# D-Hank/NeRF-tiny

Hardware: AMD Instinct MI355X
Metric: rays/sec (64 coarse + 128 fine samples), lego 400x400 (higher is better)
Workload: dtype f32

## Files before the change

### nerf-tiny_amd/csrc/field_fwd_reg.hip

```cpp
#include "field_common.h"

namespace nerf {

constexpr int RM = 32;

template <int NFT>
struct WStage {
  float4 w[NFT];
};

template <int KB, int NFT>
__device__ __forceinline__ void stage_load(const float4* __restrict__ seg_lane, int kb, WStage<NFT>& s) {
#pragma unroll
  for (int f = 0; f < NFT; ++f) s.w[f] = seg_lane[(size_t)(f * KB + kb) * 64];
}

__device__ __forceinline__ float relu1(float x) { return __int_as_float(max(__float_as_int(x), 0)); }

__device__ __forceinline__ float f4c(const float4& v, int c) { return c == 0 ? v.x : (c == 1 ? v.y : (c == 2 ? v.z : v.w)); }

struct SaveIn {
  float* rows;
  uint16_t* mask;
};

template <int KB, int NFT, int NKB, int NNFT, bool ZERO_INIT, bool RELU_IN, int SAVE = 0>
__device__ __forceinline__ void reg_layer(const int seg, const int next_seg , int lane,
                                          const f32x16* prev, f32x16* acc, WStage<8>& st0, const float* bv,
                                          const SaveIn sv, const RegBuf& rb) {
  constexpr int KT = KB / 4;
  WStage<8> st1;
  const f32x16 zero = {0.f, 0.f, 0.f, 0.f, 0.f, 0.f, 0.f, 0.f, 0.f, 0.f, 0.f, 0.f, 0.f, 0.f, 0.f, 0.f};
  if (bv != nullptr) {
    const float one_h0 = (lane < 32) ? 1.0f : 0.0f;
#pragma unroll
    for (int f = 0; f < NFT; ++f) acc[f] = __builtin_amdgcn_mfma_f32_32x32x2f32(bv[f], one_h0, zero, 0, 0, 0);
  }
  f32x16 tin[2];
  auto activate = [&](int t) {
#pragma unroll
    for (int r = 0; r < 16; ++r) tin[t & 1][r] = RELU_IN ? (SAVE == 1 ? fmaxf(prev[t][r], 0.f) : relu1(prev[t][r])) : prev[t][r];
#pragma unroll
    for (int r = 0; r < 16; ++r) asm volatile("" : "+v"(tin[t & 1][r]));
    if (SAVE == 1 || (SAVE == 2 && !RELU_IN)) {
#pragma unroll
      for (int g = 0; g < 4; ++g)
        store_row4(sv.rows + 32 * t + 8 * g, make_float4(tin[t & 1][4 * g], tin[t & 1][4 * g + 1], tin[t & 1][4 * g + 2], tin[t & 1][4 * g + 3]));
    }
    if (SAVE != 0 && RELU_IN) {
      unsigned bits = 0;
#pragma unroll
      for (int r = 0; r < 16; ++r) bits |= (prev[t][r] > 0.f) ? (1u << r) : 0u;
      sv.mask[((t & 1) * 2) * 256 + (t >> 1) * 64] = (uint16_t)bits;
    }
  };
  activate(0);
#pragma unroll
  for (int kb = 0; kb < KB; ++kb) {
    WStage<8>& ld = (kb & 1) ? st0 : st1;
    const WStage<8>& cur = (kb & 1) ? st1 : st0;
    if (kb + 1 < KB) {
#pragma unroll
      for (int f = 0; f < NFT; ++f) ld.w[f] = reg_ldw(rb, seg + (f * KB + kb + 1) * 64);
    } else if (next_seg >= 0) {
#pragma unroll
      for (int f = 0; f < NNFT; ++f) ld.w[f] = reg_ldw(rb, next_seg + (f * NKB) * 64);
    }
    __builtin_amdgcn_sched_barrier(0);
    if ((kb & 3) == 2 && (kb >> 2) + 1 < KT) activate((kb >> 2) + 1);
#pragma unroll
    for (int s = 0; s < 4; ++s) {
      const float b = tin[(kb >> 2) & 1][4 * (kb & 3) + s];
#pragma unroll
      for (int f = 0; f < NFT; ++f) {
        if (ZERO_INIT && bv == nullptr && kb == 0 && s == 0)
          acc[f] = __builtin_amdgcn_mfma_f32_32x32x2f32(f4c(cur.w[f], s), b, zero, 0, 0, 0);
        else
          acc[f] = __builtin_amdgcn_mfma_f32_32x32x2f32(f4c(cur.w[f], s), b, acc[f], 0, 0, 0);
      }
    }
  }
  if (KB & 1) st0 = st1;
}

template <int NFT>
__device__ __forceinline__ void bias_load(const float* __restrict__ bias, int lane, float (&bv)[8]) {
#pragma unroll
  for (int f = 0; f < NFT; ++f) bv[f] = bias[f * 32 + (lane & 31)];
}

#ifdef NERF_STAMPS
#define RSTAMP(slot)                                            \
  do {                                                          \
    __builtin_amdgcn_sched_barrier(0);                          \
    const unsigned long long t_ = __builtin_readcyclecounter(); \
    __builtin_amdgcn_sched_barrier(0);                          \
    tsum[slot] += t_ - tlast;                                   \
    tlast = t_;                                                 \
  } while (0)
#else
#define RSTAMP(slot) do { } while (0)
#endif

enum { SRC_RAYS = 0, SRC_POINTS = 1, SRC_LATTICE = 2 };

template <bool SAVE, bool DEBUG, int SRC = SRC_RAYS, bool RGB = true, bool GSAVE = false>
__global__ __launch_bounds__(64, 1) void k_field_fwd_reg(const FieldArgs a, const QuerySrc q) {
#ifdef NERF_STAMPS
  unsigned long long tsum[12] = {0, 0, 0, 0, 0, 0, 0, 0, 0, 0, 0, 0};
  unsigned long long tlast = __builtin_readcyclecounter();
#endif
  const int lane = threadIdx.x, j = lane & 31, h = lane >> 5;
  const int m0 = blockIdx.x * RM;
  const int m = m0 + j;
  const bool valid = m < a.M;
  const int mc = valid ? m : a.M - 1;
  const int ray = (SRC == SRC_RAYS) ? mc / a.N : mc;
  const float* rf = (SRC == SRC_RAYS) ? a.rayf + (size_t)ray * RAYF : nullptr;
  const float4* wp = a.wp;
  const RegBuf rb = reg_buf(a.wp, threadIdx.x);

  WStage<8> st0;
  stage_load<8, 8>(wp + seg_off4(SEG_L0) + lane, 0, st0);

  float p[3];
  if constexpr (SRC == SRC_RAYS) {
    sample_point(rf, a.t[mc], p);
  } else if constexpr (SRC == SRC_POINTS) {
#pragma unroll
    for (int c = 0; c < 3; ++c) p[c] = q.points[(size_t)mc * 3 + c];
  } else {
    const int iz = mc % q.nz, ixy = mc / q.nz;
    const int iy = ixy % q.ny, ix = ixy / q.ny;
    p[0] = q.lo[0] + (float)ix * q.step[0];
    p[1] = q.lo[1] + (float)iy * q.step[1];
    p[2] = q.lo[2] + (float)iz * q.step[2];
  }
  if (DEBUG && a.pts_dbg && valid && h == 0) {
    a.pts_dbg[(size_t)m * 3 + 0] = p[0];
    a.pts_dbg[(size_t)m * 3 + 1] = p[1];
    a.pts_dbg[(size_t)m * 3 + 2] = p[2];
  }
  f32x16 gp[2];
#pragma unroll
  for (int g8 = 0; g8 < 8; ++g8) {
#pragma unroll
    for (int e = 0; e < 2; ++e) {
      const int pi = 4 * g8 + 2 * h + e;
      float sv = 0.f, cv = 0.f;
      if (pi < 30) {
        const int c = pi / 10, l = pi - 10 * c;
        const float x = (c == 0) ? p[0] : ((c == 1) ? p[1] : p[2]);
        const float ph = x * __uint_as_float(kFreqPointBits[l]);
        sincos_phase(ph, sv, cv);
      }
      gp[g8 >> 2][4 * (g8 & 3) + 2 * e] = sv;
      gp[g8 >> 2][4 * (g8 & 3) + 2 * e + 1] = cv;
    }
  }
  if (DEBUG && a.gp_dbg && valid) {
#pragma unroll
    for (int g8 = 0; g8 < 8; ++g8)
#pragma unroll
      for (int s = 0; s < 4; ++s) {
        const int k = 8 * g8 + 4 * h + s;
        if (k < POINT_DIM) a.gp_dbg[(size_t)m * POINT_DIM + k] = gp[g8 >> 2][4 * (g8 & 3) + s];
      }
  }

  const size_t MS = (size_t)a.MSrows * WIDTH;
  const long long rrow = valid ? (long long)(a.row0 + m) : a.Mtot + j;
  float* const srow = SAVE ? a.save + (size_t)rrow * WIDTH + 4 * h : nullptr;
  uint16_t* const mrow = (SAVE || GSAVE) ? a.masks + ((size_t)(a.tile0 + (m0 >> 6)) * 4 + ((m0 >> 5) & 1)) * 256 + h * 32 + j : nullptr;
  const size_t MKS = (size_t)a.tiles_tot * 4 * 256;
  auto sv_rows = [&](int tensor) { return SaveIn{SAVE ? srow + (size_t)tensor * MS : nullptr, nullptr}; };
  auto sv_relu = [&](int layer) { return SaveIn{SAVE ? srow + (size_t)layer * MS : nullptr, SAVE ? mrow + (size_t)layer * MKS : nullptr}; };
  float* const gprow = GSAVE ? a.save + (size_t)rrow * QGRAD_GP + 4 * h : nullptr;
  float* const crow = GSAVE ? a.save + (size_t)a.MSrows * QGRAD_GP + (size_t)rrow * QGRAD_C + 4 * h : nullptr;
  constexpr int SV = SAVE ? 1 : (GSAVE ? 2 : 0);
  auto sv_in = [&](int layer) { return GSAVE ? SaveIn{nullptr, mrow + (size_t)layer * MKS} : sv_relu(layer); };

  RSTAMP(0);
  f32x16 A[8], B[8];
  constexpr int L256 = 8 * 32 * 64;
  constexpr int sL1 = seg_off4(SEG_L1);
  constexpr int sL5 = seg_off4(SEG_L5);
  float bv[8];

  bias_load<8>(a.w.p[B_L0], lane, bv);
  reg_layer<8, 8, 32, 8, true, false, SV>(seg_off4(SEG_L0), sL1, lane, gp, A, st0, bv, GSAVE ? SaveIn{gprow, nullptr} : sv_rows(S_GP), rb);
  RSTAMP(1);
  bias_load<8>(a.w.p[3], lane, bv);
  reg_layer<32, 8, 32, 8, true, true, SV>(sL1, sL1 + L256, lane, A, B, st0, bv, sv_in(0), rb);
  bias_load<8>(a.w.p[5], lane, bv);
  reg_layer<32, 8, 32, 8, true, true, SV>(sL1 + L256, sL1 + 2 * L256, lane, B, A, st0, bv, sv_in(1), rb);
  bias_load<8>(a.w.p[7], lane, bv);
  reg_layer<32, 8, 32, 8, true, true, SV>(sL1 + 2 * L256, seg_off4(SEG_L4A), lane, A, B, st0, bv, sv_in(2), rb);
  RSTAMP(2);
  bias_load<8>(a.w.p[9], lane, bv);
  reg_layer<32, 8, 8, 8, true, true, SV>(seg_off4(SEG_L4A), seg_off4(SEG_L4B), lane, B, A, st0, bv, sv_in(3), rb);
  reg_layer<8, 8, 32, 8, false, false>(seg_off4(SEG_L4B), sL5, lane, gp, A, st0, nullptr, SaveIn{nullptr, nullptr}, rb);
  RSTAMP(3);
  bias_load<8>(a.w.p[11], lane, bv);
  reg_layer<32, 8, 32, 8, true, true, SV>(sL5, sL5 + L256, lane, A, B, st0, bv, sv_in(4), rb);
  bias_load<8>(a.w.p[13], lane, bv);
  reg_layer<32, 8, 32, 8, true, true, SV>(sL5 + L256, sL5 + 2 * L256, lane, B, A, st0, bv, sv_in(5), rb);
  bias_load<8>(a.w.p[15], lane, bv);
  reg_layer<32, 8, 32, 4, true, true, SV>(sL5 + 2 * L256, RGB ? seg_off4(SEG_FOLD) : -1, lane, A, B, st0, bv, sv_in(6), rb);
  RSTAMP(4);
  {
    const float* ws = a.w.p[W_SIGMA] + 4 * h;
    float s = 0.f;
    float4 wq[2][4];
#pragma unroll
    for (int g = 0; g < 4; ++g) wq[0][g] = *reinterpret_cast<const float4*>(ws + 8 * g);
#pragma unroll
    for (int t = 0; t < 8; ++t) {
      if (t + 1 < 8) {
#pragma unroll
        for (int g = 0; g < 4; ++g) wq[(t + 1) & 1][g] = *reinterpret_cast<const float4*>(ws + 32 * (t + 1) + 8 * g);
      }
      if (SAVE) __builtin_amdgcn_sched_barrier(0);
      if (GSAVE) {
        unsigned bits = 0;
#pragma unroll
        for (int r = 0; r < 16; ++r) bits |= (B[t][r] > 0.f) ? (1u << r) : 0u;
        mrow[7 * MKS + ((t & 1) * 2) * 256 + (t >> 1) * 64] = (uint16_t)bits;
      }
#pragma unroll
      for (int g = 0; g < 4; ++g) {
        const float4 q = wq[t & 1][g];
        s = __builtin_fmaf(relu1(B[t][4 * g + 0]), q.x, s);
        s = __builtin_fmaf(relu1(B[t][4 * g + 1]), q.y, s);
        s = __builtin_fmaf(relu1(B[t][4 * g + 2]), q.z, s);
        s = __builtin_fmaf(relu1(B[t][4 * g + 3]), q.w, s);
      }
      if (SAVE) __builtin_amdgcn_sched_barrier(0);
    }
    s += __shfl_xor(s, 32);
    if (valid && h == 0) {
      const float pre = s + a.w.p[B_SIGMA][0];
      a.sigma[m] = fabsf(pre);
      if (SAVE || GSAVE) a.spre[a.row0 + m] = pre;
    }
  }
  RSTAMP(5);
  if constexpr (!RGB) return;
  {
    const float* dv = a.dvec + (size_t)ray * HALF + 4 * h;
#pragma unroll
    for (int f = 0; f < 4; ++f)
#pragma unroll
      for (int g = 0; g < 4; ++g) {
        const float4 q = *reinterpret_cast<const float4*>(dv + 32 * f + 8 * g);
        A[f][4 * g + 0] = q.x;
        A[f][4 * g + 1] = q.y;
        A[f][4 * g + 2] = q.z;
        A[f][4 * g + 3] = q.w;
      }
  }
  reg_layer<32, 4, 32, 4, false, true, SAVE>(seg_off4(SEG_FOLD), -1, lane, B, A, st0, nullptr, GSAVE ? SaveIn{nullptr, nullptr} : sv_relu(7), rb);
  RSTAMP(6);
  {
    const float* wc = a.w.p[W_COLOR] + 4 * h;
    float z0 = 0.f, z1 = 0.f, z2 = 0.f;
#pragma unroll
    for (int t = 0; t < 4; ++t)
#pragma unroll
      for (int g = 0; g < 4; ++g) {
        const float4 q0 = *reinterpret_cast<const float4*>(wc + 32 * t + 8 * g);
        const float4 q1 = *reinterpret_cast<const float4*>(wc + HALF + 32 * t + 8 * g);
        const float4 q2 = *reinterpret_cast<const float4*>(wc + 2 * HALF + 32 * t + 8 * g);
        const float c0 = relu1(A[t][4 * g + 0]), c1 = relu1(A[t][4 * g + 1]);
        const float c2 = relu1(A[t][4 * g + 2]), c3 = relu1(A[t][4 * g + 3]);
        if (SAVE) store_row4(srow + S_C * MS + 32 * t + 8 * g, make_float4(c0, c1, c2, c3));
        if (GSAVE) store_row4(crow + 32 * t + 8 * g, make_float4(c0, c1, c2, c3));
        z0 = __builtin_fmaf(c3, q0.w, __builtin_fmaf(c2, q0.z, __builtin_fmaf(c1, q0.y, __builtin_fmaf(c0, q0.x, z0))));
        z1 = __builtin_fmaf(c3, q1.w, __builtin_fmaf(c2, q1.z, __builtin_fmaf(c1, q1.y, __builtin_fmaf(c0, q1.x, z1))));
        z2 = __builtin_fmaf(c3, q2.w, __builtin_fmaf(c2, q2.z, __builtin_fmaf(c1, q2.y, __builtin_fmaf(c0, q2.x, z2))));
      }
    z0 += __shfl_xor(z0, 32);
    z1 += __shfl_xor(z1, 32);
    z2 += __shfl_xor(z2, 32);
    if (valid && h == 0) {
      const float* bc = a.w.p[B_COLOR];
      a.rgb[(size_t)m * 3 + 0] = 1.0f / (1.0f + expf(-(z0 + bc[0])));
      a.rgb[(size_t)m * 3 + 1] = 1.0f / (1.0f + expf(-(z1 + bc[1])));
      a.rgb[(size_t)m * 3 + 2] = 1.0f / (1.0f + expf(-(z2 + bc[2])));
    }
  }
#ifdef NERF_STAMPS
  RSTAMP(7);
  if (a.stamps && lane == 0) {
    for (int i = 0; i < 8; ++i) atomicAdd(a.stamps + i, tsum[i]);
    atomicAdd(a.stamps + 31, 1ull);
  }
#endif
}

hipError_t launch_field_fwd_reg(const FieldArgs& a, bool save, hipStream_t st) {
  const int tiles = (a.M + RM - 1) / RM;
  if (save)
    hipLaunchKernelGGL((k_field_fwd_reg<true, false>), dim3(tiles), dim3(64), 0, st, a, QuerySrc{});
  else if (a.pts_dbg || a.gp_dbg)
    hipLaunchKernelGGL((k_field_fwd_reg<false, true>), dim3(tiles), dim3(64), 0, st, a, QuerySrc{});
  else
    hipLaunchKernelGGL((k_field_fwd_reg<false, false>), dim3(tiles), dim3(64), 0, st, a, QuerySrc{});
  return hipGetLastError();
}

hipError_t launch_query_grad_fwd(const FieldArgs& a, const QuerySrc& q, bool rgb, hipStream_t st) {
  if (a.M <= 0) return hipSuccess;
  const unsigned tiles = (unsigned)(((long long)a.M + RM - 1) / RM);
  if (rgb)
    hipLaunchKernelGGL((k_field_fwd_reg<false, false, SRC_POINTS, true, true>), dim3(tiles), dim3(64), 0, st, a, q);
  else
    hipLaunchKernelGGL((k_field_fwd_reg<false, false, SRC_POINTS, false, true>), dim3(tiles), dim3(64), 0, st, a, q);
  return hipGetLastError();
}

hipError_t launch_query_reg(const FieldArgs& a, const QuerySrc& q, bool rgb, hipStream_t st) {
  if (a.M <= 0) return hipSuccess;
  const unsigned tiles = (unsigned)(((long long)a.M + RM - 1) / RM);
  if (q.points == nullptr)
    hipLaunchKernelGGL((k_field_fwd_reg<false, false, SRC_LATTICE, false>), dim3(tiles), dim3(64), 0, st, a, q);
  else if (rgb)
    hipLaunchKernelGGL((k_field_fwd_reg<false, false, SRC_POINTS, true>), dim3(tiles), dim3(64), 0, st, a, q);
  else
    hipLaunchKernelGGL((k_field_fwd_reg<false, false, SRC_POINTS, false>), dim3(tiles), dim3(64), 0, st, a, q);
  return hipGetLastError();
}

}
```

Baseline: 713,400.

## Offload ReLU to LDS atomic-max ops interleaved with MFMA chains

Replaces the VALU ReLU on layer inputs in the non-saving forward with a round-trip through LDS. Values are stored, clamped with workgroup-scope atomic max against zero, then read back. These DS ops are interleaved between MFMA instructions using sched_group_barrier, including pre-activating the head of the next layer. The aim is to take VALU work off the MFMA issue path and hide it under matrix-core latency. In exchange it adds LDS traffic, shared memory use and fragile scheduling constraints.

```diff
diff --git a/nerf-tiny_amd/csrc/field_fwd_reg.hip b/nerf-tiny_amd/csrc/field_fwd_reg.hip
--- a/nerf-tiny_amd/csrc/field_fwd_reg.hip
+++ b/nerf-tiny_amd/csrc/field_fwd_reg.hip
@@ -1,8 +1,17 @@
 #include "field_common.h"
+#include <type_traits>
 
 namespace nerf {
 
 constexpr int RM = 32;
+
+template <int I0, int I1, class F>
+__device__ __forceinline__ void static_for(F&& f) {
+  if constexpr (I0 < I1) {
+    f(std::integral_constant<int, I0>{});
+    static_for<I0 + 1, I1>(f);
+  }
+}
 
 template <int NFT>
 struct WStage {
@@ -19,16 +28,48 @@
 
 __device__ __forceinline__ float f4c(const float4& v, int c) { return c == 0 ? v.x : (c == 1 ? v.y : (c == 2 ? v.z : v.w)); }
 
+typedef int lds_i32 __attribute__((address_space(3), may_alias));
+typedef int i32x4v __attribute__((ext_vector_type(4), may_alias));
+typedef __attribute__((address_space(3))) i32x4v lds_i32x4;
+constexpr int RELU_LDS_DWORDS = 2 * 4 * 64 * 4;
+struct ReluLds {
+  lds_i32* w;
+  lds_i32* m[4];
+};
+__device__ __forceinline__ ReluLds relu_lds(lds_i32* base, int lane) {
+  ReluLds L;
+  L.w = base + 4 * lane;
+#pragma unroll
+  for (int c = 0; c < 4; ++c) L.m[c] = base + 4 * lane + ((c + (lane >> 3)) & 3);
+  return L;
+}
+template <typename DST>
+__device__ __forceinline__ void relu_lds_op(const ReluLds& L, const f32x16& src, DST& dst, int dst0, int slot, int i) {
+  const int g = i / 6, j = i - 6 * g, off = (slot * 4 + g) * 256;
+  if (j == 0) {
+    const i32x4v v = {__float_as_int(src[4 * g]), __float_as_int(src[4 * g + 1]), __float_as_int(src[4 * g + 2]), __float_as_int(src[4 * g + 3])};
+    *reinterpret_cast<lds_i32x4*>(L.w + off) = v;
+  } else if (j < 5) {
+    __hip_atomic_fetch_max(L.m[j - 1] + off, 0, __ATOMIC_RELAXED, __HIP_MEMORY_SCOPE_WORKGROUP);
+  } else {
+    const i32x4v v = *reinterpret_cast<lds_i32x4*>(L.w + off);
+#pragma unroll
+    for (int c = 0; c < 4; ++c) dst[dst0 + c] = __int_as_float(v[c]);
+  }
+}
+
 struct SaveIn {
   float* rows;
   uint16_t* mask;
 };
 
-template <int KB, int NFT, int NKB, int NNFT, bool ZERO_INIT, bool RELU_IN, int SAVE = 0>
+template <int KB, int NFT, int NKB, int NNFT, bool ZERO_INIT, bool RELU_IN, int SAVE = 0, bool LDS_RELU = false, bool NEXT_RELU = false>
 __device__ __forceinline__ void reg_layer(const int seg, const int next_seg , int lane,
                                           const f32x16* prev, f32x16* acc, WStage<8>& st0, const float* bv,
-                                          const SaveIn sv, const RegBuf& rb) {
+                                          const SaveIn sv, const RegBuf& rb, const ReluLds& rl, f32x4v& head) {
+  static_assert(!(LDS_RELU || NEXT_RELU) || SAVE != 1, "the saving forward keeps the VALU ReLU");
   constexpr int KT = KB / 4;
+  constexpr bool LR = LDS_RELU && RELU_IN;
   WStage<8> st1;
   const f32x16 zero = {0.f, 0.f, 0.f, 0.f, 0.f, 0.f, 0.f, 0.f, 0.f, 0.f, 0.f, 0.f, 0.f, 0.f, 0.f, 0.f};
   if (bv != nullptr) {
@@ -37,7 +78,31 @@
     for (int f = 0; f < NFT; ++f) acc[f] = __builtin_amdgcn_mfma_f32_32x32x2f32(bv[f], one_h0, zero, 0, 0, 0);
   }
   f32x16 tin[2];
+  if constexpr (LR) {
+#pragma unroll
+    for (int c = 0; c < 4; ++c) tin[0][c] = head[c];
+    if (bv != nullptr) {
+#pragma unroll
+      for (int i = 6; i < 14; ++i) relu_lds_op(rl, prev[0], tin[0], 4 * (i / 6), 0, i);
+#pragma unroll
+      for (int i = 6; i < 14; ++i) {
+        __builtin_amdgcn_sched_group_barrier(0x008, 1, 0);
+        __builtin_amdgcn_sched_group_barrier(0x080, 1, 0);
+      }
+    }
+  }
+  [[maybe_unused]] const int lr0 = (bv != nullptr) ? 14 : 6;
+  auto mask_word = [&](int t) {
+    unsigned bits = 0;
+#pragma unroll
+    for (int r = 0; r < 16; ++r) bits |= (prev[t][r] > 0.f) ? (1u << r) : 0u;
+    sv.mask[((t & 1) * 2) * 256 + (t >> 1) * 64] = (uint16_t)bits;
+  };
   auto activate = [&](int t) {
+    if constexpr (LR) {
+      if (SAVE != 0) mask_word(t);
+      return;
+    }
 #pragma unroll
     for (int r = 0; r < 16; ++r) tin[t & 1][r] = RELU_IN ? (SAVE == 1 ? fmaxf(prev[t][r], 0.f) : relu1(prev[t][r])) : prev[t][r];
 #pragma unroll
@@ -55,6 +120,7 @@
     }
   };
   activate(0);
+  if constexpr (!(LR || NEXT_RELU)) {
 #pragma unroll
   for (int kb = 0; kb < KB; ++kb) {
     WStage<8>& ld = (kb & 1) ? st0 : st1;
@@ -79,6 +145,57 @@
           acc[f] = __builtin_amdgcn_mfma_f32_32x32x2f32(f4c(cur.w[f], s), b, acc[f], 0, 0, 0);
       }
     }
+  }
+  } else {
+  auto ds0 = [&](int kt, int k4, int s, int f) { const int i = lr0 + (k4 * 4 + s) * NFT + f; return (LR && kt == 0 && i < 24) ? i : -1; };
+  auto ds1 = [&](int kt, int k4, int s, int f) { const int i = (k4 * 4 + s) * NFT + f - (NFT == 8 ? 64 : 16); return (LR && kt + 1 < KT && i >= 0 && i < 24) ? i : -1; };
+  auto ds2 = [&](int kt, int k4, int s, int f) { return (NEXT_RELU && kt == KT - 1 && k4 == 3 && s == 3 && f < 6) ? f : -1; };
+  static_for<0, KB>([&](auto kbc) __attribute__((always_inline)) {
+    constexpr int kb = decltype(kbc)::value, kt = kb >> 2, k4 = kb & 3;
+    WStage<8>& ld = (kb & 1) ? st0 : st1;
+    const WStage<8>& cur = (kb & 1) ? st1 : st0;
+    if (kb + 1 < KB) {
+#pragma unroll
+      for (int f = 0; f < NFT; ++f) ld.w[f] = reg_ldw(rb, seg + (f * KB + kb + 1) * 64);
+    } else if (next_seg >= 0) {
+#pragma unroll
+      for (int f = 0; f < NNFT; ++f) ld.w[f] = reg_ldw(rb, next_seg + (f * NKB) * 64);
+    }
+    __builtin_amdgcn_sched_barrier(0);
+    if (k4 == 2 && kt + 1 < KT) activate(kt + 1);
+    bool any = false;
+#pragma unroll
+    for (int s = 0; s < 4; ++s) {
+      const float b = tin[kt & 1][4 * k4 + s];
+#pragma unroll
+      for (int f = 0; f < NFT; ++f) {
+        if (ZERO_INIT && bv == nullptr && kb == 0 && s == 0)
+          acc[f] = __builtin_amdgcn_mfma_f32_32x32x2f32(f4c(cur.w[f], s), b, zero, 0, 0, 0);
+        else
+          acc[f] = __builtin_amdgcn_mfma_f32_32x32x2f32(f4c(cur.w[f], s), b, acc[f], 0, 0, 0);
+        const int i0 = ds0(kt, k4, s, f), i1 = ds1(kt, k4, s, f), i2 = ds2(kt, k4, s, f);
+        if constexpr (LR) {
+          if (i0 >= 0) relu_lds_op(rl, prev[0], tin[0], 4 * (i0 / 6), 0, i0);
+          if (i1 >= 0) relu_lds_op(rl, prev[kt + 1], tin[(kt + 1) & 1], 4 * (i1 / 6), (kt + 1) & 1, i1);
+        }
+        if constexpr (NEXT_RELU) {
+          if (i2 >= 0) relu_lds_op(rl, acc[0], head, 0, 0, i2);
+        }
+        any |= i0 >= 0 || i1 >= 0 || i2 >= 0;
+      }
+    }
+    if (any) {
+#pragma unroll
+      for (int s = 0; s < 4; ++s)
+#pragma unroll
+        for (int f = 0; f < NFT; ++f) {
+          const int n = (ds0(kt, k4, s, f) >= 0) + (ds1(kt, k4, s, f) >= 0) + (ds2(kt, k4, s, f) >= 0);
+          __builtin_amdgcn_sched_group_barrier(0x008, 1, 0);
+          if (n == 1) __builtin_amdgcn_sched_group_barrier(0x080, 1, 0);
+          if (n == 2) __builtin_amdgcn_sched_group_barrier(0x080, 2, 0);
+        }
+    }
+  });
   }
   if (KB & 1) st0 = st1;
 }
@@ -180,6 +297,13 @@
   constexpr int SV = SAVE ? 1 : (GSAVE ? 2 : 0);
   auto sv_in = [&](int layer) { return GSAVE ? SaveIn{nullptr, mrow + (size_t)layer * MKS} : sv_relu(layer); };
 
+  constexpr bool LR = !SAVE;
+  ReluLds rl{};
+  if constexpr (LR) {
+    __shared__ int relu_slots[RELU_LDS_DWORDS];
+    rl = relu_lds((lds_i32*)relu_slots, lane);
+  }
+  f32x4v head = {0.f, 0.f, 0.f, 0.f};
   RSTAMP(0);
   f32x16 A[8], B[8];
   constexpr int L256 = 8 * 32 * 64;
@@ -188,25 +312,25 @@
   float bv[8];
 
   bias_load<8>(a.w.p[B_L0], lane, bv);
-  reg_layer<8, 8, 32, 8, true, false, SV>(seg_off4(SEG_L0), sL1, lane, gp, A, st0, bv, GSAVE ? SaveIn{gprow, nullptr} : sv_rows(S_GP), rb);
+  reg_layer<8, 8, 32, 8, true, false, SV, LR, LR>(seg_off4(SEG_L0), sL1, lane, gp, A, st0, bv, GSAVE ? SaveIn{gprow, nullptr} : sv_rows(S_GP), rb, rl, head);
   RSTAMP(1);
   bias_load<8>(a.w.p[3], lane, bv);
-  reg_layer<32, 8, 32, 8, true, true, SV>(sL1, sL1 + L256, lane, A, B, st0, bv, sv_in(0), rb);
+  reg_layer<32, 8, 32, 8, true, true, SV, LR, LR>(sL1, sL1 + L256, lane, A, B, st0, bv, sv_in(0), rb, rl, head);
   bias_load<8>(a.w.p[5], lane, bv);
-  reg_layer<32, 8, 32, 8, true, true, SV>(sL1 + L256, sL1 + 2 * L256, lane, B, A, st0, bv, sv_in(1), rb);
+  reg_layer<32, 8, 32, 8, true, true, SV, LR, LR>(sL1 + L256, sL1 + 2 * L256, lane, B, A, st0, bv, sv_in(1), rb, rl, head);
   bias_load<8>(a.w.p[7], lane, bv);
-  reg_layer<32, 8, 32, 8, true, true, SV>(sL1 + 2 * L256, seg_off4(SEG_L4A), lane, A, B, st0, bv, sv_in(2), rb);
+  reg_layer<32, 8, 32, 8, true, true, SV, LR, LR>(sL1 + 2 * L256, seg_off4(SEG_L4A), lane, A, B, st0, bv, sv_in(2), rb, rl, head);
   RSTAMP(2);
   bias_load<8>(a.w.p[9], lane, bv);
-  reg_layer<32, 8, 8, 8, true, true, SV>(seg_off4(SEG_L4A), seg_off4(SEG_L4B), lane, B, A, st0, bv, sv_in(3), rb);
-  reg_layer<8, 8, 32, 8, false, false>(seg_off4(SEG_L4B), sL5, lane, gp, A, st0, nullptr, SaveIn{nullptr, nullptr}, rb);
+  reg_layer<32, 8, 8, 8, true, true, SV, LR, false>(seg_off4(SEG_L4A), seg_off4(SEG_L4B), lane, B, A, st0, bv, sv_in(3), rb, rl, head);
+  reg_layer<8, 8, 32, 8, false, false, 0, LR, LR>(seg_off4(SEG_L4B), sL5, lane, gp, A, st0, nullptr, SaveIn{nullptr, nullptr}, rb, rl, head);
   RSTAMP(3);
   bias_load<8>(a.w.p[11], lane, bv);
-  reg_layer<32, 8, 32, 8, true, true, SV>(sL5, sL5 + L256, lane, A, B, st0, bv, sv_in(4), rb);
+  reg_layer<32, 8, 32, 8, true, true, SV, LR, LR>(sL5, sL5 + L256, lane, A, B, st0, bv, sv_in(4), rb, rl, head);
   bias_load<8>(a.w.p[13], lane, bv);
-  reg_layer<32, 8, 32, 8, true, true, SV>(sL5 + L256, sL5 + 2 * L256, lane, B, A, st0, bv, sv_in(5), rb);
+  reg_layer<32, 8, 32, 8, true, true, SV, LR, LR>(sL5 + L256, sL5 + 2 * L256, lane, B, A, st0, bv, sv_in(5), rb, rl, head);
   bias_load<8>(a.w.p[15], lane, bv);
-  reg_layer<32, 8, 32, 4, true, true, SV>(sL5 + 2 * L256, RGB ? seg_off4(SEG_FOLD) : -1, lane, A, B, st0, bv, sv_in(6), rb);
+  reg_layer<32, 8, 32, 4, true, true, SV, LR, false>(sL5 + 2 * L256, RGB ? seg_off4(SEG_FOLD) : -1, lane, A, B, st0, bv, sv_in(6), rb, rl, head);
   RSTAMP(4);
   {
     const float* ws = a.w.p[W_SIGMA] + 4 * h;
@@ -259,7 +383,7 @@
         A[f][4 * g + 3] = q.w;
       }
   }
-  reg_layer<32, 4, 32, 4, false, true, SAVE>(seg_off4(SEG_FOLD), -1, lane, B, A, st0, nullptr, GSAVE ? SaveIn{nullptr, nullptr} : sv_relu(7), rb);
+  reg_layer<32, 4, 32, 4, false, true, SAVE, false, false>(seg_off4(SEG_FOLD), -1, lane, B, A, st0, nullptr, GSAVE ? SaveIn{nullptr, nullptr} : sv_relu(7), rb, rl, head);
   RSTAMP(6);
   {
     const float* wc = a.w.p[W_COLOR] + 4 * h;
```

After: 724,400, median of 6. 1.02x the previous value.
